# cisco/openh264

Measured on AMD Instinct MI355X. Metric: 1080p frames/sec/GPU at QP=24 CBP; encoder_binary_comparison SHA1 pass, higher is better.
Workload: dtype u8

## Files before the change

### openh264_amd/csrc/kernels/inter_mb.h

```cpp
#pragma once
#include "frame_kernels.h"
#include "../common/gom_rc.h"


#if defined(WH_EMU)
#include <stdio.h>
static long g_wh_win_stat[40];
static void wh_win_stat_dump() {
  if (!getenv ("WELSHIP_WIN_STATS")) return;
  fprintf (stderr, "welship mb stat: skip %ld bg/static %ld intra %ld p16x16 %ld p16x8 %ld p8x16 %ld p8x8 %ld renamed-skip %ld | searches 16x16 %ld 16x8/8x16 %ld 8x8 %ld, diamond steps %ld %ld %ld | refinements %ld %ld %ld | skip tests %ld with transform %ld\n",
           g_wh_win_stat[8], g_wh_win_stat[9], g_wh_win_stat[10], g_wh_win_stat[11], g_wh_win_stat[12], g_wh_win_stat[13], g_wh_win_stat[14], g_wh_win_stat[15], g_wh_win_stat[16], g_wh_win_stat[17], g_wh_win_stat[18],
           g_wh_win_stat[19], g_wh_win_stat[20], g_wh_win_stat[21], g_wh_win_stat[22], g_wh_win_stat[23], g_wh_win_stat[24], g_wh_win_stat[25], g_wh_win_stat[26]);
  fprintf (stderr, "welship window stat: P macroblocks %ld, reloads %ld, adopted %ld, first loads %ld, mid-walk reloads %ld, chroma predictions inside the window %ld / from the picture %ld\n", g_wh_win_stat[0], g_wh_win_stat[1], g_wh_win_stat[2], g_wh_win_stat[3], g_wh_win_stat[4], g_wh_win_stat[5], g_wh_win_stat[6]);
}
struct WhWinStatInit { WhWinStatInit() { atexit (wh_win_stat_dump); } };
static WhWinStatInit g_wh_win_stat_init;
#define WH_STAT_WIN(i) (++g_wh_win_stat[i])
#define WH_STAT_BLK(base, bw, bh) (++g_wh_win_stat[(base) + ((bw) == 16 && (bh) == 16 ? 0 : (bw) == 8 && (bh) == 8 ? 2 : 1)])
#else
#define WH_STAT_WIN(i) ((void)0)
#define WH_STAT_BLK(base, bw, bh) ((void)0)
#endif

#define WH_REF_NOT_AVAIL (-2)
#define WH_REF_NOT_IN_LIST (-1)
#define WH_WIN_STRIDE 80
#ifndef WH_WIN_ROWS
#define WH_WIN_ROWS 38
#endif
#define WH_WIN_MARGIN_X 19
#ifndef WH_WIN_MARGIN_Y
#define WH_WIN_MARGIN_Y 11
#endif
#ifndef WH_WIN_START
#define WH_WIN_START 5
#endif
#define WH_CWIN_STRIDE 64
#ifndef WH_CWIN_ROWS
#define WH_CWIN_ROWS 24
#endif
#define WH_CWIN_COLS 32

#define WH_SLOT_16x16 0
#define WH_SLOT_8x8 1
#define WH_SLOT_16x8 5
#define WH_SLOT_8x16 7

typedef struct alignas (16) WhWinLds {
  alignas (16) uint8_t win[WH_WIN_ROWS * WH_WIN_STRIDE + 16];
  alignas (16) uint8_t cwin[WH_CWIN_ROWS * WH_CWIN_STRIDE + 16];
} WhWinLds;

typedef struct alignas (16) WhInterLds {
  WhMbLds m;
  uint32_t nb[5 * 36];
  int16_t co_mv[2][2];
  uint32_t sad_cost0_in;
  int16_t mvp_out[16][2];
  int16_t mv_out[16][2];
} WhInterLds;

typedef struct alignas (16) WhInterStage {
  uint32_t cold_pv[64];
} WhInterStage;
typedef struct WhWin { int x0, y0, cx0, cy0; WhWinLds* b; } WhWin;

WH_FN int wh_se_bits (int v) {
  const unsigned k = v > 0 ? 2u * (unsigned)v : 1u - 2u * (unsigned)v;
  return 2 * (31 - __builtin_clz (k)) + 1;
}
WH_FN int wh_mvd_cost (int lambda, int dx, int dy) { return (int) (uint16_t) (lambda * wh_se_bits (dx)) + (int) (uint16_t) (lambda * wh_se_bits (dy)); }

WH_FN int wh_tap6 (int a, int b, int c, int d, int e, int f) { return a - 5 * b + 20 * c + 20 * d - 5 * e + f; }
#define WH_BYTE(v, k) ((int) (((v) >> (8 * (k))) & 255u))
WH_FN uint32_t wh_pack4 (int a, int b, int c, int d) { return (uint32_t)a | ((uint32_t)b << 8) | ((uint32_t)c << 16) | ((uint32_t)d << 24); }
WH_FN void wh_htaps4 (const uint8_t* w, int o, int* t0, int* t1, int* t2, int* t3) {
  const uint32_t a = wh_ld4u (w, o - 2), b = wh_ld4u (w, o + 2), c = wh_ld4u (w, o + 6);
  const int q0 = WH_BYTE (a, 0), q1 = WH_BYTE (a, 1), q2 = WH_BYTE (a, 2), q3 = WH_BYTE (a, 3);
  const int q4 = WH_BYTE (b, 0), q5 = WH_BYTE (b, 1), q6 = WH_BYTE (b, 2), q7 = WH_BYTE (b, 3), q8 = WH_BYTE (c, 0);
  *t0 = wh_tap6 (q0, q1, q2, q3, q4, q5); *t1 = wh_tap6 (q1, q2, q3, q4, q5, q6);
  *t2 = wh_tap6 (q2, q3, q4, q5, q6, q7); *t3 = wh_tap6 (q3, q4, q5, q6, q7, q8);
}
WH_FN uint32_t wh_mc_b4 (const uint8_t* w, int o) {
  int t0, t1, t2, t3;
  wh_htaps4 (w, o, &t0, &t1, &t2, &t3);
  return wh_pack4 (wh_clip255 ((t0 + 16) >> 5), wh_clip255 ((t1 + 16) >> 5), wh_clip255 ((t2 + 16) >> 5), wh_clip255 ((t3 + 16) >> 5));
}
WH_FN uint32_t wh_mc_h4 (const uint8_t* w, int o) {
  const uint32_t r0 = wh_ld4u (w, o - 2 * WH_WIN_STRIDE), r1 = wh_ld4u (w, o - WH_WIN_STRIDE), r2 = wh_ld4u (w, o);
  const uint32_t r3 = wh_ld4u (w, o + WH_WIN_STRIDE), r4 = wh_ld4u (w, o + 2 * WH_WIN_STRIDE), r5 = wh_ld4u (w, o + 3 * WH_WIN_STRIDE);
  int v[4];
#pragma unroll
  for (int k = 0; k < 4; ++k)
    v[k] = wh_clip255 ((wh_tap6 (WH_BYTE (r0, k), WH_BYTE (r1, k), WH_BYTE (r2, k), WH_BYTE (r3, k), WH_BYTE (r4, k), WH_BYTE (r5, k)) + 16) >> 5);
  return wh_pack4 (v[0], v[1], v[2], v[3]);
}
WH_FN uint32_t wh_mc_j4 (const uint8_t* w, int o) {
  int t[6][4];
#pragma unroll
  for (int k = 0; k < 6; ++k) wh_htaps4 (w, o + (k - 2) * WH_WIN_STRIDE, &t[k][0], &t[k][1], &t[k][2], &t[k][3]);
  int v[4];
#pragma unroll
  for (int x = 0; x < 4; ++x) v[x] = wh_clip255 ((wh_tap6 (t[0][x], t[1][x], t[2][x], t[3][x], t[4][x], t[5][x]) + 512) >> 10);
  return wh_pack4 (v[0], v[1], v[2], v[3]);
}
WH_FN uint32_t wh_mc4 (const uint8_t* w, int o, int fx, int fy) {
  switch (fy * 4 + fx) {
  case 0: return wh_ld4u (w, o);
  case 1: return wh_avg4 (wh_ld4u (w, o), wh_mc_b4 (w, o));
  case 2: return wh_mc_b4 (w, o);
  case 3: return wh_avg4 (wh_ld4u (w, o + 1), wh_mc_b4 (w, o));
  case 4: return wh_avg4 (wh_ld4u (w, o), wh_mc_h4 (w, o));
  case 5: return wh_avg4 (wh_mc_b4 (w, o), wh_mc_h4 (w, o));
  case 6: return wh_avg4 (wh_mc_b4 (w, o), wh_mc_j4 (w, o));
  case 7: return wh_avg4 (wh_mc_b4 (w, o), wh_mc_h4 (w, o + 1));
  case 8: return wh_mc_h4 (w, o);
  case 9: return wh_avg4 (wh_mc_h4 (w, o), wh_mc_j4 (w, o));
  case 10: return wh_mc_j4 (w, o);
  case 11: return wh_avg4 (wh_mc_j4 (w, o), wh_mc_h4 (w, o + 1));
  case 12: return wh_avg4 (wh_ld4u (w, o + WH_WIN_STRIDE), wh_mc_h4 (w, o));
  case 13: return wh_avg4 (wh_mc_h4 (w, o), wh_mc_b4 (w, o + WH_WIN_STRIDE));
  case 14: return wh_avg4 (wh_mc_j4 (w, o), wh_mc_b4 (w, o + WH_WIN_STRIDE));
  default: return wh_avg4 (wh_mc_h4 (w, o + 1), wh_mc_b4 (w, o + WH_WIN_STRIDE));
  }
}
WH_FN int wh_mc_chroma_w (int a, int b, int c, int d, int dx, int dy) {
  return ((8 - dx) * (8 - dy) * a + dx * (8 - dy) * b + (8 - dx) * dy * c + dx * dy * d + 32) >> 6;
}

#define WH_WIN_PIECES (WH_WIN_ROWS * (WH_WIN_STRIDE / 16))
#define WH_WIN_LOADS ((WH_WIN_PIECES + 63) / 64)
#define WH_CWIN_PIECES (WH_CWIN_ROWS * (WH_CWIN_STRIDE / 16))
#define WH_CWIN_LOADS ((WH_CWIN_PIECES + 63) / 64)
WH_FN int wh_win_pick (int lo, int hi, int align) { const int a = hi & ~ (align - 1); return a >= lo ? a : (lo + hi) >> 1; }
WH_FN void wh_win_place (const WhSeqParams& P, WhWin& W, int cx, int cy) {
  W.x0 = wh_clip3 ((cx - 24) & ~15, -32, P.mb_w * 16 + 32 - WH_WIN_STRIDE);
  W.y0 = wh_clip3 (wh_win_pick (cy + 16 + WH_WIN_MARGIN_Y - WH_WIN_ROWS, cy - WH_WIN_MARGIN_Y, 8), -32, P.mb_h * 16 + 32 - WH_WIN_ROWS);
  const int ccx = cx >> 1, ccy = cy >> 1;
  W.cx0 = wh_clip3 ((ccx - 8) & ~7, -16, P.mb_w * 8 + 16 - WH_CWIN_COLS);
  W.cy0 = wh_clip3 (wh_win_pick (ccy - (WH_CWIN_ROWS - 9) / 2 - 2, ccy - (WH_CWIN_ROWS - 9) / 2 + 1, 8), -16, P.mb_h * 8 + 16 - WH_CWIN_ROWS);
}
WH_FN uint32_t wh_tile_y_off32 (int stride_y, int x, int y) {
  return ((wh_mul_u24 ((uint32_t) ((y + 32) >> 3), (uint32_t) (stride_y >> 4)) + (uint32_t) ((x + 32) >> 4)) << 7) + (uint32_t) (((y + 32) & 7) << 4);
}
WH_FN uint32_t wh_tile_c_off32 (int stride_c, int x, int y) {
  return ((wh_mul_u24 ((uint32_t) ((y + 16) >> 3), (uint32_t) (stride_c >> 3)) + (uint32_t) ((x + 16) >> 3)) << 7) + (uint32_t) (((y + 16) & 7) << 4);
}
WH_FN const WH_G uint8_t* wh_win_src_luma (int p, const WhSeqParams& P, const WhPicJob& J, const WhWin& W) {
  const int r = (p * 205) >> 10, c = p - 5 * r;
  return (const WH_G uint8_t*)J.ref_tiles[0] + wh_tile_y_off32 (P.rec_stride_y, W.x0 + 16 * c, W.y0 + r);
}
WH_FN const WH_G uint8_t* wh_win_src_chroma (int p, const WhSeqParams& P, const WhPicJob& J, const WhWin& W) {
  return (const WH_G uint8_t*)J.ref_tiles[1] + wh_tile_c_off32 (P.rec_stride_c, W.cx0 + 8 * (p & 3), W.cy0 + (p >> 2));
}
WH_FN int wh_cwin_off (int pl, int x, int y) { return y * WH_CWIN_STRIDE + ((x >> 3) << 4) + (pl << 3) + (x & 7); }
WH_FN void wh_win_issue_luma (const WhSeqParams& P, const WhPicJob& J, WhWin& W) {
  WV_LANES_BEGIN (lane)
#pragma unroll
  for (int k = 0; k < WH_WIN_LOADS; ++k) if (64 * k + lane < WH_WIN_PIECES) wh_ld_async16 (wh_win_src_luma (64 * k + lane, P, J, W), &W.b->win[1024 * k], lane);
  WV_LANES_END
}
WH_FN void wh_win_issue_chroma (const WhSeqParams& P, const WhPicJob& J, WhWin& W) {
  WV_LANES_BEGIN (lane)
#pragma unroll
  for (int k = 0; k < WH_CWIN_LOADS; ++k) if (64 * k + lane < WH_CWIN_PIECES) wh_ld_async16 (wh_win_src_chroma (64 * k + lane, P, J, W), &W.b->cwin[1024 * k], lane);
  WV_LANES_END
}
WH_FN void wh_win_load_luma (WhInterLds& S, const WhSeqParams& P, const WhPicJob& J, WhWin& W) {
  (void)S;
  wh_win_issue_luma (P, J, W);
  WV_ASYNC_WAIT();
}
WH_FN void wh_win_issue_all (const WhSeqParams& P, const WhPicJob& J, WhWin& W, int cx, int cy) {
  wh_win_place (P, W, cx, cy);
  WV_LANES_BEGIN (lane)
  {
#pragma unroll
    for (int k = 0; k < WH_WIN_LOADS; ++k) if (64 * k + lane < WH_WIN_PIECES) wh_ld_async16 (wh_win_src_luma (64 * k + lane, P, J, W), &W.b->win[1024 * k], lane);
#pragma unroll
    for (int k = 0; k < WH_CWIN_LOADS; ++k) if (64 * k + lane < WH_CWIN_PIECES) wh_ld_async16 (wh_win_src_chroma (64 * k + lane, P, J, W), &W.b->cwin[1024 * k], lane);
  }
  WV_LANES_END
}
WH_FN bool wh_win_covers (const WhWin& W, int x0, int y0, int x1, int y1) {
  return x0 >= W.x0 && y0 >= W.y0 && x1 <= W.x0 + WH_WIN_STRIDE && y1 <= W.y0 + WH_WIN_ROWS;
}
WH_FN void wh_win_ensure (WhInterLds& S, const WhSeqParams& P, const WhPicJob& J, WhWin& W, int x0, int y0, int x1, int y1) {
  if (wh_win_covers (W, x0, y0, x1, y1)) return;
  W.x0 = wh_clip3 (wh_win_pick (x1 - WH_WIN_STRIDE, x0, 16), -32, P.mb_w * 16 + 32 - WH_WIN_STRIDE);
  W.y0 = wh_clip3 (wh_win_pick (y1 - WH_WIN_ROWS, y0, 8), -32, P.mb_h * 16 + 32 - WH_WIN_ROWS);
  WH_STAT_WIN (1);
  wh_win_load_luma (S, P, J, W);
}
WH_FN int wh_win_room (const WhWin& W, int px, int py, int bw, int bh) {
  return wh_min (wh_min (px - W.x0, W.x0 + WH_WIN_STRIDE - (px + bw + 3)), wh_min (py - W.y0, W.y0 + WH_WIN_ROWS - (py + bh)));
}
WH_FN void wh_win_need (WhInterLds& S, const WhSeqParams& P, const WhPicJob& J, WhWin& W, int px, int py, int bw, int bh, int need) {
  if (wh_win_room (W, px, py, bw, bh) >= need) return;
  wh_win_ensure (S, P, J, W, px - WH_WIN_MARGIN_X, py - WH_WIN_MARGIN_Y, px + bw + 3 + WH_WIN_MARGIN_X, py + bh + WH_WIN_MARGIN_Y);
}

WH_FN void wh_win_speculate (const WhSeqParams& P, const WhPicJob& J, WhWin& W, int mbx, int mby, int guess_mv) {
  const int gx = wh_clip3 ((2 + (int) (int16_t) (guess_mv & 0xffff)) >> 2, -P.mv_range, P.mv_range), gy = wh_clip3 ((2 + (guess_mv >> 16)) >> 2, -P.mv_range, P.mv_range);
  wh_win_issue_all (P, J, W, mbx * 16 + gx, mby * 16 + gy);
}

WH_FN int wh_sl_row (int lane, int bw) { return bw == 16 ? lane >> 2 : lane >> 1; }
WH_FN int wh_sl_col (int lane, int bw) { return bw == 16 ? (lane & 3) * 4 : (lane & 1) * 4; }
// ... 319 lines not shown
    int dx = bmx * 4 - me.mvpx, dy = bmy * 4 - me.mvpy;
    int wo = (bpy + bmy - W.y0) * WH_WIN_STRIDE + bpx + bmx - W.x0;
    const int n = (me.bw * me.bh) >> 2;
    int budget = wh_win_room (W, bpx + bmx, bpy + bmy, me.bw, me.bh);
    for (int it = 0; it < 16; ++it) {
      const int cmx = (dx + me.mvpx) >> 2, cmy = (dy + me.mvpy) >> 2;
      if (!(cmx >= C.minx && cmx < C.maxx && cmy >= C.miny && cmy < C.maxy)) break;
      if (it >= budget) {
        if (wh_win_room (W, bpx + cmx, bpy + cmy, me.bw, me.bh) < 1) {
          WH_STAT_WIN (4);
          wh_win_need (S, P, J, W, bpx + cmx, bpy + cmy, me.bw, me.bh, WH_WIN_START);
          wo = (bpy + cmy - W.y0) * WH_WIN_STRIDE + bpx + cmx - W.x0;
        }
        budget = it + wh_max (1, wh_win_room (W, bpx + cmx, bpy + cmy, me.bw, me.bh));
      }
#if defined(WH_EMU)
      if (wh_win_room (W, bpx + cmx, bpy + cmy, me.bw, me.bh) < 1 || wo != (bpy + cmy - W.y0) * WH_WIN_STRIDE + bpx + cmx - W.x0) { fprintf (stderr, "emu: diamond step outside the search window\n"); abort(); }
#endif
      WH_STAT_BLK (19, me.bw, me.bh);
      int pud, plr;
      WV_SUM2 (pud, plr, lane,
               (lane < n ? ([&] () { const int r = wh_sl_row (lane, me.bw), c = wh_sl_col (lane, me.bw);
                                     const uint32_t e = wh_enc4 (S, me.bx + c, me.by + r); const int o = wo + r * WH_WIN_STRIDE + c;
                                     return wh_sad4 (e, wh_ld4u (W.b->win, o - WH_WIN_STRIDE)) | (wh_sad4 (e, wh_ld4u (W.b->win, o + WH_WIN_STRIDE)) << 16); }) () : 0),
               (lane < n ? ([&] () { const int r = wh_sl_row (lane, me.bw), c = wh_sl_col (lane, me.bw);
                                     const uint32_t e = wh_enc4 (S, me.bx + c, me.by + r); const int o = wo + r * WH_WIN_STRIDE + c;
                                     return wh_sad4 (e, wh_ld4u (W.b->win, o - 1)) | (wh_sad4 (e, wh_ld4u (W.b->win, o + 1)) << 16); }) () : 0));
      const int c0 = (pud & 0xffff) + wh_mvd_cost (C.lambda, dx, dy - 4);
      const int c1 = (int) ((unsigned)pud >> 16) + wh_mvd_cost (C.lambda, dx, dy + 4);
      const int c2 = (plr & 0xffff) + wh_mvd_cost (C.lambda, dx - 4, dy);
      const int c3 = (int) ((unsigned)plr >> 16) + wh_mvd_cost (C.lambda, dx + 4, dy);
      const int in_cost = best;
      int ix = 0, iy = 0;
      if (c0 < best) { best = c0; ix = 0; iy = 1; }
      if (c1 < best) { best = c1; ix = 0; iy = -1; }
      if (c2 < best) { best = c2; ix = 1; iy = 0; }
      if (c3 < best) { best = c3; ix = -1; iy = 0; }
      if (best == in_cost) break;
      dx -= ix * 4; dy -= iy * 4;
      wo -= ix + iy * WH_WIN_STRIDE;
    }
    bmx = (dx + me.mvpx) >> 2; bmy = (dy + me.mvpy) >> 2;
    if (Z && Z->method >= 1) {
      if ((uint32_t)best >= Z->thr) {
        WH_STAT (WH_ST_CROSS_V);
        wh_line_search (S, P, J, W, C, me, true, &best, &bmx, &bmy);
        if ((uint32_t)best >= Z->thr) { WH_STAT (WH_ST_CROSS_H); wh_line_search (S, P, J, W, C, me, false, &best, &bmx, &bmy); }
      }
      if (Z->method == 2 && (uint32_t)best >= Z->thr) {
        const int before = best;
        WH_STAT (WH_ST_FME);
        wh_feature_search (S, P, J, Z->job, C, me, Z->thr, &best, &bmx, &bmy);
        if (best < before) WH_STAT (WH_ST_FME_HIT);
        Z->fme_down += (uint32_t) (before - best);
      }
      if (C.use_satd) wh_win_need (S, P, J, W, bpx + bmx, bpy + bmy, me.bw, me.bh, 0);
    }
  }
  me.mvx = bmx * 4; me.mvy = bmy * 4;
  me.sad_cost = best; me.satd_cost = best; me.satd_raw = 0;
  if (C.use_satd) wh_me_satd (S, W, C, me, bmx, bmy);
}

WH_FN void wh_me_fixed (WhInterLds& S, const WhSeqParams& P, const WhPicJob& J, WhWin& W, const WhMeCtx& C, WhMe& me, int imx, int imy) {
  me.sad_cost = wh_cand_sad (S, P, J, W, C, me, imx, imy) + wh_mvd_cost (C.lambda, imx * 4 - me.mvpx, imy * 4 - me.mvpy);
  me.mvx = imx * 4; me.mvy = imy * 4;
  me.satd_cost = me.sad_cost; me.satd_raw = 0;
  if (C.use_satd) {
    wh_win_need (S, P, J, W, C.mbx * 16 + me.bx + imx, C.mby * 16 + me.by + imy, me.bw, me.bh, 0);
    wh_me_satd (S, W, C, me, imx, imy);
  }
}

typedef struct WhMeTab { WvLaneArr mv, sad, satd, raw; } WhMeTab;
WH_FN void wh_me_store (WhMeTab& T, int slot, const WhMe& me) {
  WV_LSET (T.mv, slot, wh_pk_mv (me.mvx, me.mvy)); WV_LSET (T.sad, slot, me.sad_cost); WV_LSET (T.satd, slot, me.satd_cost); WV_LSET (T.raw, slot, me.satd_raw);
}
WH_FN void wh_me_fetch (const WhMeTab& T, int slot, WhMe& me) {
  const int v = WV_LGET (T.mv, slot);
  me.mvx = wh_mvx (v); me.mvy = wh_mvy (v); me.sad_cost = WV_LGET (T.sad, slot); me.satd_cost = WV_LGET (T.satd, slot); me.satd_raw = WV_LGET (T.raw, slot);
}


WH_FN void wh_rf_h_pair (const uint8_t* w, int o, uint32_t* hu, uint32_t* hd) {
  uint32_t r[7];
#pragma unroll
  for (int k = 0; k < 7; ++k) r[k] = wh_ld4u (w, o + (k - 3) * WH_WIN_STRIDE);
  int u[4], d[4];
#pragma unroll
  for (int k = 0; k < 4; ++k) {
    u[k] = wh_clip255 ((wh_tap6 (WH_BYTE (r[0], k), WH_BYTE (r[1], k), WH_BYTE (r[2], k), WH_BYTE (r[3], k), WH_BYTE (r[4], k), WH_BYTE (r[5], k)) + 16) >> 5);
    d[k] = wh_clip255 ((wh_tap6 (WH_BYTE (r[1], k), WH_BYTE (r[2], k), WH_BYTE (r[3], k), WH_BYTE (r[4], k), WH_BYTE (r[5], k), WH_BYTE (r[6], k)) + 16) >> 5);
  }
  *hu = wh_pack4 (u[0], u[1], u[2], u[3]); *hd = wh_pack4 (d[0], d[1], d[2], d[3]);
}
WH_FN void wh_htaps5 (const uint8_t* w, int o, int* t ) {
  const uint32_t a = wh_ld4u (w, o - 3), b = wh_ld4u (w, o + 1), c = wh_ld4u (w, o + 5);
  int q[10];
#pragma unroll
  for (int k = 0; k < 4; ++k) { q[k] = WH_BYTE (a, k); q[4 + k] = WH_BYTE (b, k); }
  q[8] = WH_BYTE (c, 0); q[9] = WH_BYTE (c, 1);
#pragma unroll
  for (int k = 0; k < 5; ++k) t[k] = wh_tap6 (q[k], q[k + 1], q[k + 2], q[k + 3], q[k + 4], q[k + 5]);
}
WH_FN void wh_rf_b_pair (const uint8_t* w, int o, uint32_t* bl, uint32_t* br) {
  int t[5];
  wh_htaps5 (w, o, t);
  int v[5];
#pragma unroll
  for (int k = 0; k < 5; ++k) v[k] = wh_clip255 ((t[k] + 16) >> 5);
  *bl = wh_pack4 (v[0], v[1], v[2], v[3]); *br = wh_pack4 (v[1], v[2], v[3], v[4]);
}
WH_FN void wh_rf_j_pair_h (const uint8_t* w, int o, uint32_t* jl, uint32_t* jr) {
  int t[6][5];
#pragma unroll
  for (int k = 0; k < 6; ++k) wh_htaps5 (w, o + (k - 2) * WH_WIN_STRIDE, t[k]);
  int v[5];
#pragma unroll
  for (int x = 0; x < 5; ++x) v[x] = wh_clip255 ((wh_tap6 (t[0][x], t[1][x], t[2][x], t[3][x], t[4][x], t[5][x]) + 512) >> 10);
  *jl = wh_pack4 (v[0], v[1], v[2], v[3]); *jr = wh_pack4 (v[1], v[2], v[3], v[4]);
}
WH_FN void wh_rf_j_pair_v (const uint8_t* w, int o, uint32_t* ju, uint32_t* jd) {
  int t[7][4];
#pragma unroll
  for (int k = 0; k < 7; ++k) wh_htaps4 (w, o + (k - 3) * WH_WIN_STRIDE, &t[k][0], &t[k][1], &t[k][2], &t[k][3]);
  int u[4], d[4];
#pragma unroll
  for (int x = 0; x < 4; ++x) {
    u[x] = wh_clip255 ((wh_tap6 (t[0][x], t[1][x], t[2][x], t[3][x], t[4][x], t[5][x]) + 512) >> 10);
    d[x] = wh_clip255 ((wh_tap6 (t[1][x], t[2][x], t[3][x], t[4][x], t[5][x], t[6][x]) + 512) >> 10);
  }
  *ju = wh_pack4 (u[0], u[1], u[2], u[3]); *jd = wh_pack4 (d[0], d[1], d[2], d[3]);
}
WH_FN void wh_rf_quarters (const uint8_t* w, int o, int hb, uint32_t G, uint32_t hu, uint32_t hd, uint32_t bl, uint32_t br, uint32_t* q) {
  uint32_t ja, jb;
  switch (hb) {
  case -1: q[0] = wh_avg4 (G, hu); q[1] = wh_avg4 (G, hd); q[2] = wh_avg4 (G, bl); q[3] = wh_avg4 (G, br); break;
  case 0:
    wh_rf_j_pair_h (w, o - WH_WIN_STRIDE, &ja, &jb);
    q[0] = wh_avg4 (wh_ld4u (w, o - WH_WIN_STRIDE), hu); q[1] = wh_avg4 (G, hu); q[2] = wh_avg4 (ja, hu); q[3] = wh_avg4 (jb, hu); break;
  case 1:
    wh_rf_j_pair_h (w, o, &ja, &jb);
    q[0] = wh_avg4 (G, hd); q[1] = wh_avg4 (wh_ld4u (w, o + WH_WIN_STRIDE), hd); q[2] = wh_avg4 (ja, hd); q[3] = wh_avg4 (jb, hd); break;
  case 2:
    wh_rf_j_pair_v (w, o - 1, &ja, &jb);
    q[0] = wh_avg4 (ja, bl); q[1] = wh_avg4 (jb, bl); q[2] = wh_avg4 (wh_ld4u (w, o - 1), bl); q[3] = wh_avg4 (G, bl); break;
  default:
    wh_rf_j_pair_v (w, o, &ja, &jb);
    q[0] = wh_avg4 (ja, br); q[1] = wh_avg4 (jb, br); q[2] = wh_avg4 (G, br); q[3] = wh_avg4 (wh_ld4u (w, o + 1), br); break;
  }
}

WH_FN void wh_refine_frac (WhInterLds& S, const WhSeqParams& P, const WhPicJob& J, WhWin& W, const WhMeCtx& C, WhMe& me, int satd_in_md, int sub8 = 0) {
  const int bpx = C.mbx * 16 + me.bx, bpy = C.mby * 16 + me.by;
  WH_STAT_BLK (22, me.bw, me.bh);
  const int ipx = bpx + (me.mvx >> 2), ipy = bpy + (me.mvy >> 2);
  wh_win_ensure (S, P, J, W, ipx - 4, ipy - 4, ipx + me.bw + 8, ipy + me.bh + 5);
  const int wo = (ipy - W.y0) * WH_WIN_STRIDE + ipx - W.x0;
  const int nq = (me.bw >> 2) * (me.bh >> 2) * 4, bw = me.bw, ex = me.bx, ey = me.by;
#define WH_RF_ACT (lane < nq && (!sub8 || (bw == 16 ? ((lane >> 2) & 3) < 2 : lane < 16)))
#define WH_RF_ENC wh_enc4 (S, ex + (lane < nq ? wh_tl_col (lane, bw) : 0), ey + (lane < nq ? wh_tl_row (lane, bw) : 0))
#define WH_RF_O (wo + (lane < nq ? wh_tl_row (lane, bw) * WH_WIN_STRIDE + wh_tl_col (lane, bw) : 0))
  const int dmx = me.mvx - me.mvpx, dmy = me.mvy - me.mvpy;
  WvLaneArr vG, vhu, vhd, vbl, vbr, vq0, vq1, vq2, vq3;
#if defined(WH_EMU)
  memset (&vG, 0, sizeof (vG)); memset (&vhu, 0, sizeof (vhu)); memset (&vhd, 0, sizeof (vhd)); memset (&vbl, 0, sizeof (vbl)); memset (&vbr, 0, sizeof (vbr));
  memset (&vq0, 0, sizeof (vq0)); memset (&vq1, 0, sizeof (vq1)); memset (&vq2, 0, sizeof (vq2)); memset (&vq3, 0, sizeof (vq3));
#else
  vG = 0; vhu = 0; vhd = 0; vbl = 0; vbr = 0; vq0 = 0; vq1 = 0; vq2 = 0; vq3 = 0;
#endif
  int c_int, c0, c1, c2, c3;
  WV_DECLARE_LANE (lane);
  WV_LANE_EVAL (lane, {
    const int o = WH_RF_O;
    uint32_t a, b;
    WV_LOWN (vG, lane) = (int)wh_ld4u (W.b->win, o);
    wh_rf_h_pair (W.b->win, o, &a, &b); WV_LOWN (vhu, lane) = (int)a; WV_LOWN (vhd, lane) = (int)b;
    wh_rf_b_pair (W.b->win, o, &a, &b); WV_LOWN (vbl, lane) = (int)a; WV_LOWN (vbr, lane) = (int)b; });
  if (satd_in_md) c_int = me.satd_raw;
  else WV_SATD_ROWS_SHARED (c_int, lane, WH_RF_ACT, WH_RF_ENC, (uint32_t)WV_LOWN (vG, lane));
  WV_SATD_ROWS4_SHARED (c0, c1, c2, c3, lane, WH_RF_ACT, WH_RF_ENC, (uint32_t)WV_LOWN (vhu, lane), (uint32_t)WV_LOWN (vhd, lane), (uint32_t)WV_LOWN (vbl, lane), (uint32_t)WV_LOWN (vbr, lane));
  int best = c_int + wh_mvd_cost (C.lambda, dmx, dmy), hb = -1;
  c0 += wh_mvd_cost (C.lambda, dmx, dmy - 2); if (c0 < best) { best = c0; hb = 0; }
  c1 += wh_mvd_cost (C.lambda, dmx, dmy + 2); if (c1 < best) { best = c1; hb = 1; }
  c2 += wh_mvd_cost (C.lambda, dmx - 2, dmy); if (c2 < best) { best = c2; hb = 2; }
  c3 += wh_mvd_cost (C.lambda, dmx + 2, dmy); if (c3 < best) { best = c3; hb = 3; }
  const int hx = hb == 2 ? -2 : hb == 3 ? 2 : 0, hy = hb == 0 ? -2 : hb == 1 ? 2 : 0;
  WV_LANE_EVAL (lane, {
    uint32_t q[4];
    wh_rf_quarters (W.b->win, WH_RF_O, hb, (uint32_t)WV_LOWN (vG, lane), (uint32_t)WV_LOWN (vhu, lane), (uint32_t)WV_LOWN (vhd, lane), (uint32_t)WV_LOWN (vbl, lane), (uint32_t)WV_LOWN (vbr, lane), q);
    WV_LOWN (vq0, lane) = (int)q[0]; WV_LOWN (vq1, lane) = (int)q[1]; WV_LOWN (vq2, lane) = (int)q[2]; WV_LOWN (vq3, lane) = (int)q[3]; });
  WV_SATD_ROWS4_SHARED (c0, c1, c2, c3, lane, WH_RF_ACT, WH_RF_ENC, (uint32_t)WV_LOWN (vq0, lane), (uint32_t)WV_LOWN (vq1, lane), (uint32_t)WV_LOWN (vq2, lane), (uint32_t)WV_LOWN (vq3, lane));
  int qb = -1;
  c0 += wh_mvd_cost (C.lambda, dmx + hx, dmy + hy - 1); if (c0 < best) { best = c0; qb = 0; }
  c1 += wh_mvd_cost (C.lambda, dmx + hx, dmy + hy + 1); if (c1 < best) { best = c1; qb = 1; }
  c2 += wh_mvd_cost (C.lambda, dmx + hx - 1, dmy + hy); if (c2 < best) { best = c2; qb = 2; }
  c3 += wh_mvd_cost (C.lambda, dmx + hx + 1, dmy + hy); if (c3 < best) { best = c3; qb = 3; }
  const int qx = qb == 2 ? -1 : qb == 3 ? 1 : 0, qy = qb == 0 ? -1 : qb == 1 ? 1 : 0;
  me.satd_cost = best;
  WV_LANE_EVAL (lane, {
    if (lane < nq) {
      const int v = qb >= 0 ? (qb == 0 ? WV_LOWN (vq0, lane) : qb == 1 ? WV_LOWN (vq1, lane) : qb == 2 ? WV_LOWN (vq2, lane) : WV_LOWN (vq3, lane))
                  : hb >= 0 ? (hb == 0 ? WV_LOWN (vhu, lane) : hb == 1 ? WV_LOWN (vhd, lane) : hb == 2 ? WV_LOWN (vbl, lane) : WV_LOWN (vbr, lane)) : WV_LOWN (vG, lane);
      * (uint32_t*)&S.m.pred_y[(ey + wh_tl_row (lane, bw)) * 16 + ex + wh_tl_col (lane, bw)] = (uint32_t)v;
    } });
  WV_SYNC();
#undef WH_RF_ACT
#undef WH_RF_ENC
#undef WH_RF_O
  me.mvx += hx + qx; me.mvy += hy + qy;
}

WH_FN int wh_enc_inter_y (WhMbLds& S, int qp) {
  wh_quant_blocks (S, 0, 16, qp, qp, S.res, 0);
  int s0, s1, s2, s3;
  WV_QUADSUM4 (s0, s1, s2, s3, lane, (lane < 16 ? WH_Q_SCORE (S.part2[lane]) : 0));
  int cbp = 0;
  if (s0 + s1 + s2 + s3 >= 6) cbp = (s0 >= 4 ? 1 : 0) | (s1 >= 4 ? 2 : 0) | (s2 >= 4 ? 4 : 0) | (s3 >= 4 ? 8 : 0);
  WV_LANES_BEGIN (lane)
  {
    const int b = lane >> 2, on = (cbp >> (b >> 2)) & 1;
    for (int q = 0; q < 4; ++q) { const int k = (lane & 3) * 4 + q; S.lv_luma[b * 16 + k] = S.res[b * 16 + wh_zigzag (k)]; }
    if (lane < 16) {
      int n = 0;
      if ((cbp >> (lane >> 2)) & 1) n = __builtin_popcount (WH_Q_MASK (S.part2[lane]));
      S.nzc[wh_blk_y (lane) * 4 + wh_blk_x (lane)] = (uint8_t)n;
    }
    (void)on;
  }
  WV_LANES_END
  WV_LANES_BEGIN (lane)
  {
    const int b = lane >> 2, on = (cbp >> (b >> 2)) & 1;
    for (int k = 0; k < 4; ++k) {
      const int i = lane * 4 + k, pos = i & 15;
      S.res[i] = on ? (int16_t) (S.res[i] * wh_dq (qp, pos)) : (int16_t)0;
    }
  }
  WV_LANES_END
  return cbp;
}

WH_FN bool wh_try_py_skip (WhMbLds& S, int qp) {
  wh_quant_blocks (S, 0, 16, qp, qp, S.tmp, 0);
  int bc, u1, u2, u3;
  WV_ROWSUM4 (bc, u1, u2, u3, lane, (lane < 16 ? WH_Q_SCORE (S.part2[lane]) | (WH_Q_BIG (S.part2[lane]) << 16) : 0));
  (void)u1; (void)u2; (void)u3;
  return bc < 6;
}
WH_FN bool wh_try_puv_skip (WhMbLds& S, int qpc) {
  const int ff = wh_ff_inter (qpc, 0) << 1, mf = wh_mf (qpc, 0) >> 1;
  const int16_t thr = (int16_t) (((1 << 16) - 1) / mf - ff);
  for (int pl = 0; pl < 2; ++pl) {
    const int16_t* r = &S.res[256 + pl * 64];
    const int16_t s0 = (int16_t) (r[0] + r[32]), s1 = (int16_t) (r[0] - r[32]), s2 = (int16_t) (r[16] + r[48]), s3 = (int16_t) (r[16] - r[48]);
    const int16_t d0 = (int16_t) (s0 + s2), d1 = (int16_t) (s0 - s2), d2 = (int16_t) (s1 + s3), d3 = (int16_t) (s1 - s3);
    if (wh_abs (d0) > thr || wh_abs (d1) > thr || wh_abs (d2) > thr || wh_abs (d3) > thr) return false;
  }
  wh_quant_blocks (S, 256, 8, qpc, qpc, S.tmp, 1);
  int c0, c1, c2, c3;
  WV_QUADSUM4 (c0, c1, c2, c3, lane, (lane < 8 ? WH_Q_SCORE (S.part2[lane]) | (WH_Q_BIG (S.part2[lane]) << 8) : 0));
// ... 691 lines not shown
```

Baseline: 27780.

## Rewrite luma six-tap interpolation with packed dot4/dot2 and 16-bit SIMD ops

```diff
diff --git a/openh264_amd/csrc/kernels/inter_mb.h b/openh264_amd/csrc/kernels/inter_mb.h
--- a/openh264_amd/csrc/kernels/inter_mb.h
+++ b/openh264_amd/csrc/kernels/inter_mb.h
@@ -1,5 +1,6 @@
 #pragma once
 #include "frame_kernels.h"
+#include "luma_interp.h"
 #include "../common/gom_rc.h"
 
 
@@ -71,59 +72,8 @@
 }
 WH_FN int wh_mvd_cost (int lambda, int dx, int dy) { return (int) (uint16_t) (lambda * wh_se_bits (dx)) + (int) (uint16_t) (lambda * wh_se_bits (dy)); }
 
-WH_FN int wh_tap6 (int a, int b, int c, int d, int e, int f) { return a - 5 * b + 20 * c + 20 * d - 5 * e + f; }
-#define WH_BYTE(v, k) ((int) (((v) >> (8 * (k))) & 255u))
 WH_FN uint32_t wh_pack4 (int a, int b, int c, int d) { return (uint32_t)a | ((uint32_t)b << 8) | ((uint32_t)c << 16) | ((uint32_t)d << 24); }
-WH_FN void wh_htaps4 (const uint8_t* w, int o, int* t0, int* t1, int* t2, int* t3) {
-  const uint32_t a = wh_ld4u (w, o - 2), b = wh_ld4u (w, o + 2), c = wh_ld4u (w, o + 6);
-  const int q0 = WH_BYTE (a, 0), q1 = WH_BYTE (a, 1), q2 = WH_BYTE (a, 2), q3 = WH_BYTE (a, 3);
-  const int q4 = WH_BYTE (b, 0), q5 = WH_BYTE (b, 1), q6 = WH_BYTE (b, 2), q7 = WH_BYTE (b, 3), q8 = WH_BYTE (c, 0);
-  *t0 = wh_tap6 (q0, q1, q2, q3, q4, q5); *t1 = wh_tap6 (q1, q2, q3, q4, q5, q6);
-  *t2 = wh_tap6 (q2, q3, q4, q5, q6, q7); *t3 = wh_tap6 (q3, q4, q5, q6, q7, q8);
-}
-WH_FN uint32_t wh_mc_b4 (const uint8_t* w, int o) {
-  int t0, t1, t2, t3;
-  wh_htaps4 (w, o, &t0, &t1, &t2, &t3);
-  return wh_pack4 (wh_clip255 ((t0 + 16) >> 5), wh_clip255 ((t1 + 16) >> 5), wh_clip255 ((t2 + 16) >> 5), wh_clip255 ((t3 + 16) >> 5));
-}
-WH_FN uint32_t wh_mc_h4 (const uint8_t* w, int o) {
-  const uint32_t r0 = wh_ld4u (w, o - 2 * WH_WIN_STRIDE), r1 = wh_ld4u (w, o - WH_WIN_STRIDE), r2 = wh_ld4u (w, o);
-  const uint32_t r3 = wh_ld4u (w, o + WH_WIN_STRIDE), r4 = wh_ld4u (w, o + 2 * WH_WIN_STRIDE), r5 = wh_ld4u (w, o + 3 * WH_WIN_STRIDE);
-  int v[4];
-#pragma unroll
-  for (int k = 0; k < 4; ++k)
-    v[k] = wh_clip255 ((wh_tap6 (WH_BYTE (r0, k), WH_BYTE (r1, k), WH_BYTE (r2, k), WH_BYTE (r3, k), WH_BYTE (r4, k), WH_BYTE (r5, k)) + 16) >> 5);
-  return wh_pack4 (v[0], v[1], v[2], v[3]);
-}
-WH_FN uint32_t wh_mc_j4 (const uint8_t* w, int o) {
-  int t[6][4];
-#pragma unroll
-  for (int k = 0; k < 6; ++k) wh_htaps4 (w, o + (k - 2) * WH_WIN_STRIDE, &t[k][0], &t[k][1], &t[k][2], &t[k][3]);
-  int v[4];
-#pragma unroll
-  for (int x = 0; x < 4; ++x) v[x] = wh_clip255 ((wh_tap6 (t[0][x], t[1][x], t[2][x], t[3][x], t[4][x], t[5][x]) + 512) >> 10);
-  return wh_pack4 (v[0], v[1], v[2], v[3]);
-}
-WH_FN uint32_t wh_mc4 (const uint8_t* w, int o, int fx, int fy) {
-  switch (fy * 4 + fx) {
-  case 0: return wh_ld4u (w, o);
-  case 1: return wh_avg4 (wh_ld4u (w, o), wh_mc_b4 (w, o));
-  case 2: return wh_mc_b4 (w, o);
-  case 3: return wh_avg4 (wh_ld4u (w, o + 1), wh_mc_b4 (w, o));
-  case 4: return wh_avg4 (wh_ld4u (w, o), wh_mc_h4 (w, o));
-  case 5: return wh_avg4 (wh_mc_b4 (w, o), wh_mc_h4 (w, o));
-  case 6: return wh_avg4 (wh_mc_b4 (w, o), wh_mc_j4 (w, o));
-  case 7: return wh_avg4 (wh_mc_b4 (w, o), wh_mc_h4 (w, o + 1));
-  case 8: return wh_mc_h4 (w, o);
-  case 9: return wh_avg4 (wh_mc_h4 (w, o), wh_mc_j4 (w, o));
-  case 10: return wh_mc_j4 (w, o);
-  case 11: return wh_avg4 (wh_mc_j4 (w, o), wh_mc_h4 (w, o + 1));
-  case 12: return wh_avg4 (wh_ld4u (w, o + WH_WIN_STRIDE), wh_mc_h4 (w, o));
-  case 13: return wh_avg4 (wh_mc_h4 (w, o), wh_mc_b4 (w, o + WH_WIN_STRIDE));
-  case 14: return wh_avg4 (wh_mc_j4 (w, o), wh_mc_b4 (w, o + WH_WIN_STRIDE));
-  default: return wh_avg4 (wh_mc_h4 (w, o + 1), wh_mc_b4 (w, o + WH_WIN_STRIDE));
-  }
-}
+WH_FN uint32_t wh_mc4 (const uint8_t* w, int o, int fx, int fy) { return wh_li_mc4 (w, o, WH_WIN_STRIDE, fx, fy); }
 WH_FN int wh_mc_chroma_w (int a, int b, int c, int d, int dx, int dy) {
   return ((8 - dx) * (8 - dy) * a + dx * (8 - dy) * b + (8 - dx) * dy * c + dx * dy * d + 32) >> 6;
 }
@@ -609,71 +559,21 @@
 }
 
 
-WH_FN void wh_rf_h_pair (const uint8_t* w, int o, uint32_t* hu, uint32_t* hd) {
-  uint32_t r[7];
-#pragma unroll
-  for (int k = 0; k < 7; ++k) r[k] = wh_ld4u (w, o + (k - 3) * WH_WIN_STRIDE);
-  int u[4], d[4];
-#pragma unroll
-  for (int k = 0; k < 4; ++k) {
-    u[k] = wh_clip255 ((wh_tap6 (WH_BYTE (r[0], k), WH_BYTE (r[1], k), WH_BYTE (r[2], k), WH_BYTE (r[3], k), WH_BYTE (r[4], k), WH_BYTE (r[5], k)) + 16) >> 5);
-    d[k] = wh_clip255 ((wh_tap6 (WH_BYTE (r[1], k), WH_BYTE (r[2], k), WH_BYTE (r[3], k), WH_BYTE (r[4], k), WH_BYTE (r[5], k), WH_BYTE (r[6], k)) + 16) >> 5);
-  }
-  *hu = wh_pack4 (u[0], u[1], u[2], u[3]); *hd = wh_pack4 (d[0], d[1], d[2], d[3]);
-}
-WH_FN void wh_htaps5 (const uint8_t* w, int o, int* t ) {
-  const uint32_t a = wh_ld4u (w, o - 3), b = wh_ld4u (w, o + 1), c = wh_ld4u (w, o + 5);
-  int q[10];
-#pragma unroll
-  for (int k = 0; k < 4; ++k) { q[k] = WH_BYTE (a, k); q[4 + k] = WH_BYTE (b, k); }
-  q[8] = WH_BYTE (c, 0); q[9] = WH_BYTE (c, 1);
-#pragma unroll
-  for (int k = 0; k < 5; ++k) t[k] = wh_tap6 (q[k], q[k + 1], q[k + 2], q[k + 3], q[k + 4], q[k + 5]);
-}
-WH_FN void wh_rf_b_pair (const uint8_t* w, int o, uint32_t* bl, uint32_t* br) {
-  int t[5];
-  wh_htaps5 (w, o, t);
-  int v[5];
-#pragma unroll
-  for (int k = 0; k < 5; ++k) v[k] = wh_clip255 ((t[k] + 16) >> 5);
-  *bl = wh_pack4 (v[0], v[1], v[2], v[3]); *br = wh_pack4 (v[1], v[2], v[3], v[4]);
-}
-WH_FN void wh_rf_j_pair_h (const uint8_t* w, int o, uint32_t* jl, uint32_t* jr) {
-  int t[6][5];
-#pragma unroll
-  for (int k = 0; k < 6; ++k) wh_htaps5 (w, o + (k - 2) * WH_WIN_STRIDE, t[k]);
-  int v[5];
-#pragma unroll
-  for (int x = 0; x < 5; ++x) v[x] = wh_clip255 ((wh_tap6 (t[0][x], t[1][x], t[2][x], t[3][x], t[4][x], t[5][x]) + 512) >> 10);
-  *jl = wh_pack4 (v[0], v[1], v[2], v[3]); *jr = wh_pack4 (v[1], v[2], v[3], v[4]);
-}
-WH_FN void wh_rf_j_pair_v (const uint8_t* w, int o, uint32_t* ju, uint32_t* jd) {
-  int t[7][4];
-#pragma unroll
-  for (int k = 0; k < 7; ++k) wh_htaps4 (w, o + (k - 3) * WH_WIN_STRIDE, &t[k][0], &t[k][1], &t[k][2], &t[k][3]);
-  int u[4], d[4];
-#pragma unroll
-  for (int x = 0; x < 4; ++x) {
-    u[x] = wh_clip255 ((wh_tap6 (t[0][x], t[1][x], t[2][x], t[3][x], t[4][x], t[5][x]) + 512) >> 10);
-    d[x] = wh_clip255 ((wh_tap6 (t[1][x], t[2][x], t[3][x], t[4][x], t[5][x], t[6][x]) + 512) >> 10);
-  }
-  *ju = wh_pack4 (u[0], u[1], u[2], u[3]); *jd = wh_pack4 (d[0], d[1], d[2], d[3]);
-}
 WH_FN void wh_rf_quarters (const uint8_t* w, int o, int hb, uint32_t G, uint32_t hu, uint32_t hd, uint32_t bl, uint32_t br, uint32_t* q) {
   uint32_t ja, jb;
   switch (hb) {
   case -1: q[0] = wh_avg4 (G, hu); q[1] = wh_avg4 (G, hd); q[2] = wh_avg4 (G, bl); q[3] = wh_avg4 (G, br); break;
   case 0:
-    wh_rf_j_pair_h (w, o - WH_WIN_STRIDE, &ja, &jb);
+    wh_li_j_pair_h (w, o - WH_WIN_STRIDE, WH_WIN_STRIDE, &ja, &jb);
     q[0] = wh_avg4 (wh_ld4u (w, o - WH_WIN_STRIDE), hu); q[1] = wh_avg4 (G, hu); q[2] = wh_avg4 (ja, hu); q[3] = wh_avg4 (jb, hu); break;
   case 1:
-    wh_rf_j_pair_h (w, o, &ja, &jb);
+    wh_li_j_pair_h (w, o, WH_WIN_STRIDE, &ja, &jb);
     q[0] = wh_avg4 (G, hd); q[1] = wh_avg4 (wh_ld4u (w, o + WH_WIN_STRIDE), hd); q[2] = wh_avg4 (ja, hd); q[3] = wh_avg4 (jb, hd); break;
   case 2:
-    wh_rf_j_pair_v (w, o - 1, &ja, &jb);
+    wh_li_j_pair_v (w, o - 1, WH_WIN_STRIDE, &ja, &jb);
     q[0] = wh_avg4 (ja, bl); q[1] = wh_avg4 (jb, bl); q[2] = wh_avg4 (wh_ld4u (w, o - 1), bl); q[3] = wh_avg4 (G, bl); break;
   default:
-    wh_rf_j_pair_v (w, o, &ja, &jb);
+    wh_li_j_pair_v (w, o, WH_WIN_STRIDE, &ja, &jb);
     q[0] = wh_avg4 (ja, br); q[1] = wh_avg4 (jb, br); q[2] = wh_avg4 (G, br); q[3] = wh_avg4 (wh_ld4u (w, o + 1), br); break;
   }
 }
@@ -702,8 +602,8 @@
     const int o = WH_RF_O;
     uint32_t a, b;
     WV_LOWN (vG, lane) = (int)wh_ld4u (W.b->win, o);
-    wh_rf_h_pair (W.b->win, o, &a, &b); WV_LOWN (vhu, lane) = (int)a; WV_LOWN (vhd, lane) = (int)b;
-    wh_rf_b_pair (W.b->win, o, &a, &b); WV_LOWN (vbl, lane) = (int)a; WV_LOWN (vbr, lane) = (int)b; });
+    wh_li_h_pair (W.b->win, o, WH_WIN_STRIDE, &a, &b); WV_LOWN (vhu, lane) = (int)a; WV_LOWN (vhd, lane) = (int)b;
+    wh_li_b_pair (W.b->win, o, &a, &b); WV_LOWN (vbl, lane) = (int)a; WV_LOWN (vbr, lane) = (int)b; });
   if (satd_in_md) c_int = me.satd_raw;
   else WV_SATD_ROWS_SHARED (c_int, lane, WH_RF_ACT, WH_RF_ENC, (uint32_t)WV_LOWN (vG, lane));
   WV_SATD_ROWS4_SHARED (c0, c1, c2, c3, lane, WH_RF_ACT, WH_RF_ENC, (uint32_t)WV_LOWN (vhu, lane), (uint32_t)WV_LOWN (vhd, lane), (uint32_t)WV_LOWN (vbl, lane), (uint32_t)WV_LOWN (vbr, lane));
diff --git a/openh264_amd/csrc/kernels/luma_interp.h b/openh264_amd/csrc/kernels/luma_interp.h
--- /dev/null
+++ b/openh264_amd/csrc/kernels/luma_interp.h
@@ -0,0 +1,168 @@
+#pragma once
+#include "wave.h"
+
+#if defined(WH_EMU)
+WH_FN uint32_t wh_perm (uint32_t hi, uint32_t lo, uint32_t sel) {
+  const uint64_t v = ((uint64_t)hi << 32) | lo;
+  uint32_t r = 0;
+  for (int k = 0; k < 4; ++k) {
+    const uint32_t s = (sel >> (8 * k)) & 255u;
+    r |= (s < 8 ? (uint32_t) (v >> (8 * s)) & 255u : 0u) << (8 * k);
+  }
+  return r;
+}
+WH_FN uint32_t wh_udot4 (uint32_t a, uint32_t b, uint32_t c) {
+  for (int k = 0; k < 4; ++k) c += ((a >> (8 * k)) & 255u) * ((b >> (8 * k)) & 255u);
+  return c;
+}
+WH_FN int wh_sdot2 (uint32_t a, uint32_t b, int c) {
+  return (int) ((uint32_t)c + (uint32_t) ((int)(int16_t)a * (int)(int16_t)b) + (uint32_t) ((int)(int16_t) (a >> 16) * (int)(int16_t) (b >> 16)));
+}
+WH_FN uint32_t wh_pk16 (int lo, int hi) { return (uint32_t) (uint16_t)lo | ((uint32_t) (uint16_t)hi << 16); }
+WH_FN uint32_t wh_pk_add (uint32_t a, uint32_t b) { return wh_pk16 ((int16_t)a + (int16_t)b, (int16_t) (a >> 16) + (int16_t) (b >> 16)); }
+WH_FN uint32_t wh_pk_mad (uint32_t a, int k, uint32_t c) { return wh_pk16 ((int16_t)a * k + (int16_t)c, (int16_t) (a >> 16) * k + (int16_t) (c >> 16)); }
+WH_FN uint32_t wh_pk_rclip (uint32_t a, int r, int n) {
+  const int lo = (int16_t) ((int16_t)a + r) >> n, hi = (int16_t) ((int16_t) (a >> 16) + r) >> n;
+  return wh_pk16 (lo < 0 ? 0 : lo > 255 ? 255 : lo, hi < 0 ? 0 : hi > 255 ? 255 : hi);
+}
+#else
+WH_FN uint32_t wh_perm (uint32_t hi, uint32_t lo, uint32_t sel) { return __builtin_amdgcn_perm (hi, lo, sel); }
+WH_FN uint32_t wh_udot4 (uint32_t a, uint32_t b, uint32_t c) { return __builtin_amdgcn_udot4 (a, b, c, false); }
+WH_FN int wh_sdot2 (uint32_t a, uint32_t b, int c) { return __builtin_amdgcn_sdot2 (wh_as_s16x2 (a), wh_as_s16x2 (b), c, false); }
+WH_FN uint32_t wh_pk_add (uint32_t a, uint32_t b) { return wh_as_u32 (wh_as_s16x2 (a) + wh_as_s16x2 (b)); }
+WH_FN uint32_t wh_pk_mad (uint32_t a, int k, uint32_t c) { const wh_s16x2 kk = {(short)k, (short)k}; return wh_as_u32 (wh_as_s16x2 (a) * kk + wh_as_s16x2 (c)); }
+WH_FN uint32_t wh_pk_rclip (uint32_t a, int r, int n) {
+  const wh_s16x2 rr = {(short)r, (short)r}, nn = {(short)n, (short)n}, z = {0, 0}, m = {255, 255};
+  return wh_as_u32 (__builtin_elementwise_min (__builtin_elementwise_max ((wh_as_s16x2 (a) + rr) >> nn, z), m));
+}
+#endif
+
+WH_FN uint32_t wh_li_ld (const uint8_t* w, int o, int d) {
+#if defined(WH_EMU)
+  return wh_ld4u (w, o + d);
+#else
+  const uint32_t* p = (const uint32_t*)w + (o >> 2) + (d >> 2);
+  return __builtin_amdgcn_alignbyte (p[1], p[0], (uint32_t)o & 3u);
+#endif
+}
+
+#define WH_LI_W1 0x01141401u
+#define WH_LI_W5L 0x00000505u
+#define WH_LI_W5H 0x05050000u
+template <int N>
+WH_FN void wh_li_hsums (uint32_t a, uint32_t b, uint32_t c, uint32_t bias, uint32_t* t) {
+  const uint32_t n01 = ~wh_perm (b, a, 0x05020401u), n23 = ~wh_perm (b, a, 0x07040603u);
+  bias -= 2550u;
+  t[0] = wh_udot4 (n01, WH_LI_W5L, wh_udot4 (wh_perm (b, a, 0x05030200u), WH_LI_W1, bias));
+  t[1] = wh_udot4 (n01, WH_LI_W5H, wh_udot4 (wh_perm (b, a, 0x06040301u), WH_LI_W1, bias));
+  t[2] = wh_udot4 (n23, WH_LI_W5L, wh_udot4 (wh_perm (b, a, 0x07050402u), WH_LI_W1, bias));
+  t[3] = wh_udot4 (n23, WH_LI_W5H, wh_udot4 (wh_perm (b, a, 0x0c060503u) | (c << 24), WH_LI_W1, bias));
+  if (N > 4) t[4] = wh_udot4 (~wh_perm (c, b, 0x0c0c0401u), WH_LI_W5L, wh_udot4 (wh_perm (c, b, 0x05030200u), WH_LI_W1, bias));
+}
+WH_FN uint32_t wh_li_pack_b (const uint32_t* t) {
+  return wh_perm (wh_pk_rclip (wh_perm (t[3], t[2], 0x05040100u), 0, 5), wh_pk_rclip (wh_perm (t[1], t[0], 0x05040100u), 0, 5), 0x06040200u);
+}
+
+#define WH_LI_C01 0x0c010c00u
+#define WH_LI_C23 0x0c030c02u
+WH_FN uint32_t wh_li_vpair (const uint32_t* r, uint32_t sel) {
+  uint32_t s = wh_perm (0u, r[0], sel);
+  s = wh_pk_mad (wh_perm (0u, r[1], sel), -5, s);
+  s = wh_pk_mad (wh_perm (0u, r[2], sel), 20, s);
+  s = wh_pk_mad (wh_perm (0u, r[3], sel), 20, s);
+  s = wh_pk_mad (wh_perm (0u, r[4], sel), -5, s);
+  return wh_pk_add (wh_perm (0u, r[5], sel), s);
+}
+WH_FN uint32_t wh_li_v4 (const uint32_t* r) {
+  return wh_perm (wh_pk_rclip (wh_li_vpair (r, WH_LI_C23), 16, 5), wh_pk_rclip (wh_li_vpair (r, WH_LI_C01), 16, 5), 0x06040200u);
+}
+WH_FN void wh_li_vcols (const uint8_t* w, int o, int st, uint32_t* v ) {
+  uint32_t a[6], b[6], c[6];
+#pragma unroll
+  for (int k = 0; k < 6; ++k) { const int d = (k - 2) * st; a[k] = wh_li_ld (w, o, d); b[k] = wh_li_ld (w, o, d + 4); c[k] = wh_li_ld (w, o, d + 8); }
+  v[0] = wh_li_vpair (a, WH_LI_C01); v[1] = wh_li_vpair (a, WH_LI_C23);
+  v[2] = wh_li_vpair (b, WH_LI_C01); v[3] = wh_li_vpair (b, WH_LI_C23);
+  v[4] = wh_li_vpair (c, WH_LI_C01);
+}
+#define WH_LI_P(lo, hi) ((uint32_t) (uint16_t) (lo) | ((uint32_t) (uint16_t) (hi) << 16))
+WH_FN int wh_li_j_even (const uint32_t* v) {
+  return wh_clip255 (wh_sdot2 (v[2], WH_LI_P (-5, 1), wh_sdot2 (v[1], WH_LI_P (20, 20), wh_sdot2 (v[0], WH_LI_P (1, -5), 512))) >> 10);
+}
+WH_FN int wh_li_j_odd (const uint32_t* v) {
+  return wh_clip255 (wh_sdot2 (v[3], WH_LI_P (1, 0), wh_sdot2 (v[2], WH_LI_P (20, -5), wh_sdot2 (v[1], WH_LI_P (-5, 20), wh_sdot2 (v[0], WH_LI_P (0, 1), 512)))) >> 10);
+}
+WH_FN uint32_t wh_li_pack4 (int a, int b, int c, int d) { return (uint32_t)a | ((uint32_t)b << 8) | ((uint32_t)c << 16) | ((uint32_t)d << 24); }
+WH_FN uint32_t wh_li_j4 (const uint32_t* v) {
+  return wh_li_pack4 (wh_li_j_even (v), wh_li_j_odd (v), wh_li_j_even (v + 1), wh_li_j_odd (v + 1));
+}
+
+WH_FN uint32_t wh_li_b4 (const uint8_t* w, int o) {
+  uint32_t t[4];
+  wh_li_hsums<4> (wh_li_ld (w, o - 2, 0), wh_li_ld (w, o - 2, 4), wh_li_ld (w, o - 2, 8), 16u, t);
+  return wh_li_pack_b (t);
+}
+WH_FN uint32_t wh_li_h4 (const uint8_t* w, int o, int st) {
+  uint32_t r[6];
+#pragma unroll
+  for (int k = 0; k < 6; ++k) r[k] = wh_li_ld (w, o, (k - 2) * st);
+  return wh_li_v4 (r);
+}
+WH_FN uint32_t wh_li_j4_at (const uint8_t* w, int o, int st) {
+  uint32_t v[5];
+  wh_li_vcols (w, o - 2, st, v);
+  return wh_li_j4 (v);
+}
+WH_FN uint32_t wh_li_h4_of (const uint32_t* v, int shift) {
+  const uint32_t h1 = wh_pk_rclip (v[1], 16, 5), h2 = wh_pk_rclip (v[2], 16, 5);
+  return shift ? wh_perm (h2, h1, 0x0c060402u) | (wh_pk_rclip (v[3], 16, 5) << 24) : wh_perm (h2, h1, 0x06040200u);
+}
+
+WH_FN uint32_t wh_li_mc4 (const uint8_t* w, int o, int st, int fx, int fy) {
+  switch (fy * 4 + fx) {
+  case 0: return wh_ld4u (w, o);
+  case 1: return wh_avg4 (wh_ld4u (w, o), wh_li_b4 (w, o));
+  case 2: return wh_li_b4 (w, o);
+  case 3: return wh_avg4 (wh_ld4u (w, o + 1), wh_li_b4 (w, o));
+  case 4: return wh_avg4 (wh_ld4u (w, o), wh_li_h4 (w, o, st));
+  case 5: return wh_avg4 (wh_li_b4 (w, o), wh_li_h4 (w, o, st));
+  case 6: return wh_avg4 (wh_li_b4 (w, o), wh_li_j4_at (w, o, st));
+  case 7: return wh_avg4 (wh_li_b4 (w, o), wh_li_h4 (w, o + 1, st));
+  case 8: return wh_li_h4 (w, o, st);
+  case 9: case 11: {
+    uint32_t v[5];
+    wh_li_vcols (w, o - 2, st, v);
+    return wh_avg4 (wh_li_j4 (v), wh_li_h4_of (v, fx == 3));
+  }
+  case 10: return wh_li_j4_at (w, o, st);
+  case 12: return wh_avg4 (wh_ld4u (w, o + st), wh_li_h4 (w, o, st));
+  case 13: return wh_avg4 (wh_li_h4 (w, o, st), wh_li_b4 (w, o + st));
+  case 14: return wh_avg4 (wh_li_j4_at (w, o, st), wh_li_b4 (w, o + st));
+  default: return wh_avg4 (wh_li_h4 (w, o + 1, st), wh_li_b4 (w, o + st));
+  }
+}
+
+WH_FN void wh_li_h_pair (const uint8_t* w, int o, int st, uint32_t* hu, uint32_t* hd) {
+  uint32_t r[7];
+#pragma unroll
+  for (int k = 0; k < 7; ++k) r[k] = wh_li_ld (w, o, (k - 3) * st);
+  *hu = wh_li_v4 (r); *hd = wh_li_v4 (r + 1);
+}
+WH_FN void wh_li_b_pair (const uint8_t* w, int o, uint32_t* bl, uint32_t* br) {
+  uint32_t t[5];
+  wh_li_hsums<5> (wh_li_ld (w, o - 3, 0), wh_li_ld (w, o - 3, 4), wh_li_ld (w, o - 3, 8), 16u, t);
+  *bl = wh_li_pack_b (t);
+  *br = wh_funnel4 (*bl, (uint32_t)wh_clip255 ((int)t[4] >> 5), 1);
+}
+WH_FN void wh_li_j_pair_h (const uint8_t* w, int o, int st, uint32_t* jl, uint32_t* jr) {
+  uint32_t v[5];
+  wh_li_vcols (w, o - 3, st, v);
+  const int j0 = wh_li_j_even (v), j1 = wh_li_j_odd (v), j2 = wh_li_j_even (v + 1), j3 = wh_li_j_odd (v + 1), j4 = wh_li_j_even (v + 2);
+  *jl = wh_li_pack4 (j0, j1, j2, j3); *jr = wh_li_pack4 (j1, j2, j3, j4);
+}
+WH_FN void wh_li_j_pair_v (const uint8_t* w, int o, int st, uint32_t* ju, uint32_t* jd) {
+  uint32_t v[5];
+  wh_li_vcols (w, o - 2 - st, st, v);
+  *ju = wh_li_j4 (v);
+  wh_li_vcols (w, o - 2, st, v);
+  *jd = wh_li_j4 (v);
+}
```

Result: no change. 27930, median of 6 (+0.5%).
